# rohanpsingh/LearningHumanoidWalking

Measured on AMD Instinct MI355X. Metric: env-steps/s (whole job): on-device rollout + GAE + PPO update, higher is better.
Workload: dtype f64 physics / f32 networks

## Files before the change

include/lhw.h:

```cpp
#ifndef LHW_H
#define LHW_H

#include <stdint.h>

#include "lhw_model_fields.h"

#ifdef __cplusplus
extern "C" {
#endif

typedef enum {
  LHW_OK = 0,
  LHW_ERR_ARG = -1,
  LHW_ERR_HIP = -2,
  LHW_ERR_MODEL = -3,
  LHW_ERR_UNSUPPORTED = -4,
  LHW_ERR_NO_DEVICE = -5
} LhwStatus;

typedef enum {
  LHW_TASK_CARTPOLE = 0,
  LHW_TASK_JVRC_WALK = 1,
  LHW_TASK_H1_STAND = 2,
  LHW_TASK_JVRC_STEP = 3,
// ... 279 lines not shown
                       int64_t ws_row, float* mu, float* act, float* logp, float* value, void* stream);
int lhw_ppo_set_inference_dtype(LhwPpo* ppo, int fp16);
int lhw_ppo_set_update_dtype(LhwPpo* ppo, int fp16);
int lhw_ppo_debug_set_strip_fused(LhwPpo* ppo, int32_t on);
int lhw_ppo_debug_set_strip_wide(LhwPpo* ppo, int32_t on);
int lhw_ppo_debug_set_strip_fp16(LhwPpo* ppo, int32_t on);
int lhw_ppo_debug_last_grad_fused(const LhwPpo* ppo);
int lhw_ppo_debug_plan(const LhwPpo* ppo, int32_t B, int32_t imitation, int32_t* out13);
int lhw_gae(int32_t T, int32_t N, const float* rew, const float* val, const uint8_t* done, const float* vterm,
            const float* vfinal, double gamma, double lam, float* ret, float* adv, void* stream);
int lhw_moments(const float* x, int64_t n, double* out2_dev, void* stream);
int lhw_scale_shift(float* x, int64_t n, float mean, float inv_scale, void* stream);
int lhw_standardize(float* x, int64_t n, const double* stats3_dev, double eps, void* stream);
int lhw_ppo_set_imitation(LhwPpo* ppo, const float* target, const uint8_t* mask, float coeff, int64_t n_selected);
int lhw_ppo_grad(LhwPpo* ppo, const float* theta, float* grad, const float* xn, const float* xm, const float* act,
                 const float* old_logp, const float* adv, const float* ret, const int32_t* idx, int32_t B,
                 float* stats_dev, void* stream);
int lhw_ppo_apply(LhwPpo* ppo, float* theta, float* grad, float* adam_m, float* adam_v, int64_t step, float grad_scale,
                  void* stream);
int lhw_ppo_debug_grad_sqnorms(LhwPpo* ppo, float* out2_host);
int lhw_ppo_step(LhwPpo* ppo, float* theta, float* grad, float* adam_m, float* adam_v, const float* xn, const float* xm, const float* act,
                 const float* old_logp, const float* adv, const float* ret, const int32_t* idx, int32_t B, float* stats_dev, int64_t step,
                 float grad_scale, void* stream);

typedef struct LhwRnn LhwRnn;
int lhw_rnn_create(const LhwPpoConfig* cfg, int32_t seq_len, int32_t seq_cols, int32_t rollout_rows, LhwRnn** out);
int lhw_rnn_destroy(LhwRnn* rnn);
int64_t lhw_rnn_param_count(const LhwRnn* rnn);
int lhw_rnn_layout(const LhwRnn* rnn, int64_t* out19);
int lhw_rnn_forward(LhwRnn* rnn, const float* theta, const float* obs, int64_t N, const float* obs_mean, const float* obs_std,
                    const uint8_t* reset, uint64_t seed, uint32_t env_id_base, uint32_t counter, int deterministic, int commit,
                    float* mu, float* act, float* logp, float* value, void* stream);
int lhw_rnn_values(LhwRnn* rnn, const float* theta, const float* obs, const float* term_obs, const uint8_t* done,
                   const uint8_t* reset0, int32_t T, int32_t N, const float* obs_mean, const float* obs_std,
                   float* val, float* vterm, float* vfinal, void* stream);
int lhw_rnn_rollout_policy(LhwRnn* rnn, const float* theta, const float* obs_mean, const float* obs_std, uint64_t seed, uint32_t counter,
                           int deterministic, LhwRolloutLstmPolicy* out, void* stream);
int lhw_rnn_grad(LhwRnn* rnn, const float* theta, float* grad, int32_t T, int32_t N, const float* xn, const float* xm,
                 const float* act, const float* old_logp, const float* adv, const float* ret, const uint8_t* done,
                 const int32_t* cols, int32_t B, float* stats_dev, void* stream);
int lhw_rnn_apply(LhwRnn* rnn, float* theta, float* grad, float* adam_m, float* adam_v, int64_t step, float grad_scale,
                  void* stream);
#define LHW_LSTM_SEQ_MIN_HIDDEN 32
#define LHW_LSTM_SEQ_MAX_HIDDEN 256
#define LHW_LSTM_SEQ_MAX_OBS_PAD 128
#define LHW_ROLLOUT_HISTORY_MAX_OBS_PAD 1024
// ... 38 lines not shown
```

learninghumanoidwalking_amd/_lib.py:

```python
from __future__ import annotations

import ctypes
import glob
import os
import subprocess

import numpy as np

_HERE = os.path.dirname(os.path.abspath(__file__))
_ROOT = os.path.dirname(_HERE)
LIB_PATH = os.environ.get("LHW_LIB") or os.path.join(_HERE, "liblhw.so")
_LIB = None


class LhwError(RuntimeError):
    def __init__(self, code, msg):
        super().__init__(f"liblhw error {code}: {msg}")
        self.code = code


class LhwEnvConfig(ctypes.Structure):
    _fields_ = [
        ("task", ctypes.c_int32), ("n_envs", ctypes.c_int32), ("device", ctypes.c_int32),
        ("frame_skip", ctypes.c_int32), ("max_traj_len", ctypes.c_int32), ("env_id_base", ctypes.c_int32),
# ... 324 lines not shown
    sig("lhw_ppo_debug_last_grad_fused", [vp])
    sig("lhw_ppo_debug_plan", [vp, i32, i32, ctypes.POINTER(i32)])
    sig("lhw_debug_wgrad_wide", [vp, vp, i32, i32, vp, vp, vp])
    sig("lhw_debug_wgrad_skinny", [i32, i32, i32, i32, vp, vp, i32, vp, vp, i32, vp, vp, vp, vp, vp, vp])
    sig("lhw_debug_dpp_forms", [u64, vp, vp, vp, vp])
    sig("lhw_debug_fastmath", [i64, vp, vp, vp, vp, vp, vp, vp])
    sig("lhw_env_phase_cycles", [vp, ctypes.c_int, vp])
    sig("lhw_env_step_range", [vp, i32, i32, vp, vp, vp, vp, vp, vp, vp])
    sig("lhw_ppo_create", [ctypes.POINTER(LhwPpoConfig), ctypes.POINTER(vp)])
    sig("lhw_ppo_destroy", [vp])
    sig("lhw_ppo_param_count", [vp], i64)
    sig("lhw_ppo_layout", [vp, ctypes.POINTER(i64)])
    sig("lhw_ppo_normalize", [vp, vp, i64, vp, vp, vp, vp, vp])
    sig("lhw_ppo_forward", [vp, vp, vp, i64, vp, vp, u64, u32, u32, ctypes.c_int, vp, vp, vp, vp, vp])
    sig("lhw_ppo_forward_at", [vp, vp, vp, i64, vp, vp, u64, u32, u32, ctypes.c_int, i64, vp, vp, vp, vp, vp])
    sig("lhw_ppo_begin_rollout", [vp, vp, vp])
    sig("lhw_ppo_end_rollout", [vp])
    sig("lhw_ppo_set_inference_dtype", [vp, ctypes.c_int])
    sig("lhw_ppo_set_update_dtype", [vp, ctypes.c_int])
    sig("lhw_ppo_set_imitation", [vp, vp, vp, f32, i64])
    sig("lhw_ppo_grad", [vp, vp, vp, vp, vp, vp, vp, vp, vp, vp, i32, vp, vp])
    sig("lhw_ppo_apply", [vp, vp, vp, vp, vp, i64, f32, vp])
    sig("lhw_ppo_step", [vp, vp, vp, vp, vp, vp, vp, vp, vp, vp, vp, vp, i32, vp, i64, f32, vp])
    sig("lhw_ppo_debug_grad_sqnorms", [vp, ctypes.POINTER(f32)])
    sig("lhw_gae", [i32, i32, vp, vp, vp, vp, vp, ctypes.c_double, ctypes.c_double, vp, vp, vp])
    sig("lhw_moments", [vp, i64, vp, vp])
    sig("lhw_scale_shift", [vp, i64, f32, f32, vp])
    sig("lhw_standardize", [vp, i64, vp, ctypes.c_double, vp])
    sig("lhw_rnn_create", [ctypes.POINTER(LhwPpoConfig), i32, i32, i32, ctypes.POINTER(vp)])
    sig("lhw_rnn_destroy", [vp])
    sig("lhw_rnn_param_count", [vp], i64)
    sig("lhw_rnn_layout", [vp, ctypes.POINTER(i64)])
    sig("lhw_rnn_normalize", [vp, vp, i64, vp, vp, vp, vp, vp])
    sig("lhw_rnn_forward", [vp, vp, vp, i64, vp, vp, vp, u64, u32, u32, ctypes.c_int, ctypes.c_int, vp, vp, vp, vp, vp])
    sig("lhw_rnn_grad", [vp, vp, vp, i32, i32, vp, vp, vp, vp, vp, vp, vp, vp, i32, vp, vp])
    sig("lhw_rnn_apply", [vp, vp, vp, vp, vp, i64, f32, vp])
    sig("lhw_rnn_debug_grad_sqnorms", [vp, ctypes.POINTER(f32)])
    sig("lhw_rnn_debug_set_seq_fused", [vp, i32])
    sig("lhw_rnn_debug_last_grad_fused", [vp])
    sig("lhw_debug_lstm_seq", [ctypes.POINTER(LhwLstmSeqArgs), i32, vp])
    sig("lhw_debug_lstm_values", [ctypes.POINTER(LhwLstmValuesArgs), i32, vp])
    sig("lhw_rnn_values", [vp, vp, vp, vp, vp, vp, i32, i32, vp, vp, vp, vp, vp, vp])
    sig("lhw_env_debug_step_record", [vp, vp, vp, vp])
    sig("lhw_env_rollout", [vp, ctypes.POINTER(LhwRolloutPolicy), i32, i32, i32, vp, vp, vp, vp, vp, vp, vp, vp])
    sig("lhw_env_last_rollout_queued", [vp])
    sig("lhw_env_rollout_task_inputs", [vp, ctypes.POINTER(LhwRolloutPolicy), i32, i32, i32, vp, vp, vp, vp, vp, vp, vp, vp, vp])
# ... 39 lines not shown
```

learninghumanoidwalking_amd/csrc/lhw_learner.h:

```cpp
#pragma once
#include "lhw_internal.h"

struct LearnerCore {
  int device = 0, D = 0, Dp = 0, A = 0, H = 0, learn_std = 0;
  float clip, ent_coeff, mirror_coeff, grad_clip, lr, adam_eps, beta1, beta2;
  int use_mirror = 0;
  size_t off_actor = 0, off_std = 0, off_critic = 0, n_critic = 0, n_params = 0;
  int *d_obs_src = nullptr, *d_act_src = nullptr;
  float *d_obs_sign = nullptr, *d_act_sign = nullptr;
  float *stats = nullptr;
  float *stats_part = nullptr;
  float *norm_part = nullptr;
  LhwDevMem mem;
};
#define SUMSQ_BLOCKS 128

int learner_check(const LhwPpoConfig* c, void** out, bool caps_ok);
void learner_init(LearnerCore& k, const LhwPpoConfig* c, size_t n_actor, size_t n_critic);
bool learner_mirror(LearnerCore& k, const LhwPpoConfig* c);
int learner_normalize(LearnerCore* k, const float* obs, int64_t R, const float* obs_mean, const float* obs_std, float* xn, float* xm, void* stream);
int learner_apply(LearnerCore* k, float* theta, float* grad, float* adam_m, float* adam_v, int64_t step, float grad_scale, void* stream);
int learner_grad_sqnorms(LearnerCore* k, float* out2_host);

struct AdamArgs {
  float *theta, *grad, *m, *v;
  size_t n0, off1, n1;
  int blocks0;
  float gscale;
  float* part;
  float* normsq_out;
  float max_norm, lr, beta1, beta2, eps, bc1, bc2sqrt;
};
AdamArgs learner_adam_args(const LearnerCore& k, float* theta, float* grad, float* adam_m, float* adam_v, int64_t step, float grad_scale);
__global__ void adam2_kernel(AdamArgs a);

struct StreamPair {
  hipStream_t s, sc;
  hipEvent_t ev_fork, ev_join;
  void fork() const { if (sc != s) { (void)hipEventRecord(ev_fork, s); (void)hipStreamWaitEvent(sc, ev_fork, 0); } }
  void join() const { if (sc != s) { (void)hipEventRecord(ev_join, sc); (void)hipStreamWaitEvent(s, ev_join, 0); } }
};

__global__ void normalize_kernel(const float* __restrict__ obs, int D, int Dp, size_t R, const float* __restrict__ mean, const float* __restrict__ stdv,
                                 float* __restrict__ xn, float* __restrict__ xm, const int* __restrict__ src, const float* __restrict__ sign);
__global__ void sample_kernel(const float* __restrict__ mu, int ldmu, int A, int N, const float* __restrict__ stdv, uint64_t seed, uint32_t env_base,
                              uint32_t counter, int deterministic, float* __restrict__ act, float* __restrict__ logp);
__global__ void ppo_loss_kernel(int B, int Rcap, int A, int Op, const float* __restrict__ ya, const float* __restrict__ yc, const float* __restrict__ act,
                                const float* __restrict__ old_logp, const float* __restrict__ adv, const float* __restrict__ ret,
                                const float* __restrict__ stdv, float clip, float mirror_coeff, int use_mirror, const int* __restrict__ act_src,
                                const float* __restrict__ act_sign, float* __restrict__ dya, float* __restrict__ dyc, float* __restrict__ dstd,
                                float* __restrict__ stats_part, const float* __restrict__ imit_target, const unsigned char* __restrict__ imit_mask,
                                float imit_coeff, float imit_inv_count, int seqB, float gscale);
__global__ void ppo_stats_rows_kernel(int B, int A, const float* __restrict__ rows, int ld, float imit_inv_count, float* __restrict__ stats_part);
__global__ void reduce_rows_kernel(const float* __restrict__ part, int nrows, int n, float* __restrict__ out);
__global__ void entropy_grad_kernel(const float* __restrict__ stdv, int A, float ent_coeff, float* __restrict__ grad_std);
```

learninghumanoidwalking_amd/csrc/lhw_learner.hip:

```cpp
#include "lhw_learner.h"

#include <cmath>
#include <mutex>
#include <vector>

#include "lhw_policy.h"
#include "lhw_rng.h"

__global__ void normalize_kernel(const float* __restrict__ obs, int D, int Dp, size_t R, const float* __restrict__ mean,
                                 const float* __restrict__ stdv, float* __restrict__ xn, float* __restrict__ xm,
                                 const int* __restrict__ src, const float* __restrict__ sign) {
  size_t i = (size_t)blockIdx.x * blockDim.x + threadIdx.x;
  if (i >= R * (size_t)Dp) return;
  size_t r = i / Dp;
  int j = (int)(i - r * Dp);
  float v = 0.f, vm = 0.f;
  if (j < D) {
    v = (obs[r * D + j] - mean[j]) / stdv[j];
    if (xm) vm = (sign[j] * obs[r * D + src[j]] - mean[j]) / stdv[j];
  }
  xn[i] = v;
  if (xm) xm[i] = vm;
}
__global__ void __launch_bounds__(256) sample_kernel(const float* __restrict__ mu, int ldmu, int A, int N, const float* __restrict__ stdv,
// ... 59 lines not shown
                                                             float* __restrict__ stats_part) {
  const int m = blockIdx.x * blockDim.x + threadIdx.x;
  float t[NSTAT] = {0, 0, 0, 0, 0, 0};
  if (m < B)
    for (int k = 0; k < NSTAT; k++) t[k] = rows[(size_t)k * ld + m];
  const float invB = 1.f / (float)B, invBA = 1.f / ((float)B * (float)A);
  float vals[NSTAT] = {t[0] * invB, t[1] * invB, t[2] * invBA, t[3] * invB, t[4] * invB, t[5] * imit_inv_count};
  ppo_stats_block(vals, stats_part);
}

__global__ void reduce_rows_kernel(const float* __restrict__ part, int nrows, int n, float* __restrict__ out) {
  int k = threadIdx.x;
  if (k >= n) return;
  float s = 0.f;
  for (int b = 0; b < nrows; b++) s += part[(size_t)b * n + k];
  out[k] += s;
}

__global__ void entropy_grad_kernel(const float* __restrict__ stdv, int A, float ent_coeff, float* __restrict__ grad_std) {
  int a = threadIdx.x;
  if (a < A) grad_std[a] += -ent_coeff / ((float)A * stdv[a]);
}
__global__ void __launch_bounds__(256) sumsq2_kernel(const float* __restrict__ g0, size_t n0, const float* __restrict__ g1, size_t n1, float scale,
                                                     float* __restrict__ part ) {
  const int grp = blockIdx.x / SUMSQ_BLOCKS, b = blockIdx.x - grp * SUMSQ_BLOCKS;
  const float* __restrict__ g = grp ? g1 : g0;
  const size_t n = grp ? n1 : n0;
  float s = 0.f;
  for (size_t i = (size_t)b * blockDim.x + threadIdx.x; i < n; i += (size_t)SUMSQ_BLOCKS * blockDim.x) {
    float v = g[i] * scale;
    s += v * v;
  }
  for (int o = 32; o > 0; o >>= 1) s += __shfl_xor(s, o);
  __shared__ float red[4];
  LHW_LDS_POISON(red);
  if ((threadIdx.x & 63) == 0) red[threadIdx.x >> 6] = s;
  __syncthreads();
  if (threadIdx.x == 0) part[blockIdx.x] = (red[0] + red[1]) + (red[2] + red[3]);
}
__global__ void __launch_bounds__(256) adam2_kernel(AdamArgs a) {
  float *__restrict__ theta = a.theta, *__restrict__ grad = a.grad, *__restrict__ m = a.m, *__restrict__ v = a.v, *__restrict__ normsq_out = a.normsq_out;
  const float* __restrict__ part = a.part;
  const size_t n0 = a.n0, off1 = a.off1, n1 = a.n1;
  const int blocks0 = a.blocks0;
  const float gscale = a.gscale, max_norm = a.max_norm, lr = a.lr, beta1 = a.beta1, beta2 = a.beta2, eps = a.eps, bc1 = a.bc1, bc2sqrt = a.bc2sqrt;
  const int grp = (int)blockIdx.x >= blocks0 ? 1 : 0;
  __shared__ float nsq;
  LHW_LDS_POISON(nsq);
  if (threadIdx.x == 0) {
    float s = 0.f;
    for (int b = 0; b < SUMSQ_BLOCKS; b++) s += part[grp * SUMSQ_BLOCKS + b];
    nsq = s;
    if ((int)blockIdx.x == (grp ? blocks0 : 0)) normsq_out[grp] = s;
  }
  __syncthreads();
  const size_t i = (size_t)((int)blockIdx.x - (grp ? blocks0 : 0)) * blockDim.x + threadIdx.x;
  if (i >= (grp ? n1 : n0)) return;
  const size_t e = (grp ? off1 : 0) + i;
  float norm = sqrtf(nsq);
  float coef = max_norm / (norm + 1e-6f);
  coef = coef < 1.f ? coef : 1.f;
  float g = grad[e] * gscale * coef;
  float mi = beta1 * m[e] + (1.f - beta1) * g;
  float vi = beta2 * v[e] + (1.f - beta2) * g * g;
  m[e] = mi; v[e] = vi;
  float denom = sqrtf(vi) / bc2sqrt + eps;
  theta[e] -= (lr / bc1) * (mi / denom);
  grad[e] = 0.f;
}
__global__ void __launch_bounds__(256) gae_kernel(int T, int N, const float* __restrict__ rew, const float* __restrict__ val,
                                                  const uint8_t* __restrict__ done, const float* __restrict__ vterm,
                                                  const float* __restrict__ vfinal, double gamma, double lam,
                                                  float* __restrict__ ret, float* __restrict__ adv) {
  int n = blockIdx.x * blockDim.x + threadIdx.x;
  if (n >= N) return;
  double gae = 0.0, nextv = (double)vfinal[n];
  for (int t = T - 1; t >= 0; t--) {
    size_t i = (size_t)t * N + n;
    uint8_t f = done[i];
// ... 124 lines not shown
  return LHW_OK;
}
extern "C" int lhw_scale_shift(float* x, int64_t n, float mean, float inv_scale, void* stream) {
  if (!x || n <= 0) return lhw_fail(LHW_ERR_ARG, "bad argument");
  int dev = 0;
  if (device_of(x, &dev)) return LHW_ERR_HIP;
  hipLaunchKernelGGL(scale_shift_kernel, dim3((n + 255) / 256), dim3(256), 0, (hipStream_t)stream, x, (size_t)n, mean, inv_scale);
  HIPCHK(hipGetLastError());
  return LHW_OK;
}

extern "C" int lhw_standardize(float* x, int64_t n, const double* stats3_dev, double eps, void* stream) {
  if (!x || !stats3_dev || n <= 0) return lhw_fail(LHW_ERR_ARG, "bad argument");
  int dev = 0;
  if (device_of(x, &dev)) return LHW_ERR_HIP;
  hipLaunchKernelGGL(standardize_kernel, dim3((n + 255) / 256), dim3(256), 0, (hipStream_t)stream, x, (size_t)n, stats3_dev, eps);
  HIPCHK(hipGetLastError());
  return LHW_OK;
}
AdamArgs learner_adam_args(const LearnerCore& k, float* theta, float* grad, float* adam_m, float* adam_v, int64_t step, float grad_scale) {
  const size_t na = k.learn_std ? k.off_std + k.A : k.off_std;
  const float bc1 = 1.f - powf(k.beta1, (float)step), bc2 = 1.f - powf(k.beta2, (float)step);
  return AdamArgs{theta, grad, adam_m, adam_v, na, k.off_critic, k.n_critic, (int)((na + 255) / 256), grad_scale, k.norm_part, k.stats + 8,
                  k.grad_clip, k.lr, k.beta1, k.beta2, k.adam_eps, bc1, sqrtf(bc2)};
}
static void clip_and_adam(const AdamArgs& a, hipStream_t s) {
  const int blocks1 = (int)((a.n1 + 255) / 256);
  hipLaunchKernelGGL(sumsq2_kernel, dim3(2 * SUMSQ_BLOCKS), dim3(256), 0, s, a.grad, a.n0, a.grad + a.off1, a.n1, a.gscale, a.part);
  hipLaunchKernelGGL(adam2_kernel, dim3(a.blocks0 + blocks1), dim3(256), 0, s, a);
}

int learner_apply(LearnerCore* k, float* theta, float* grad, float* adam_m, float* adam_v, int64_t step, float grad_scale, void* stream) {
  if (!k || !theta || !grad || !adam_m || !adam_v || step <= 0) return lhw_fail(LHW_ERR_ARG, "bad argument");
  HIPCHK(hipSetDevice(k->device));
  hipStream_t s = (hipStream_t)stream;
  clip_and_adam(learner_adam_args(*k, theta, grad, adam_m, adam_v, step, grad_scale), s);
  if (!k->learn_std) HIPCHK(hipMemsetAsync(grad + k->off_std, 0, sizeof(float) * pad4(k->A), s));
  HIPCHK(hipGetLastError());
  return LHW_OK;
}

int learner_grad_sqnorms(LearnerCore* k, float* out2_host) {
  if (!k || !out2_host) return lhw_fail(LHW_ERR_ARG, "null argument");
  HIPCHK(hipSetDevice(k->device));
  HIPCHK(hipDeviceSynchronize());
  HIPCHK(hipMemcpy(out2_host, k->stats + 8, 2 * sizeof(float), hipMemcpyDeviceToHost));
  return LHW_OK;
}
```

learninghumanoidwalking_amd/csrc/lhw_ppo.hip:

```cpp
#include <hip/hip_runtime.h>

#include <cmath>
#include <cstdlib>
#include <cstring>
#include <memory>
#include <vector>

#include "lhw_gemm.h"
#include "lhw_learner.h"
#include "lhw_mlp_strip_h.h"

struct MlpLayout {
  int D, Dp, H, O, Op;
  size_t w1, b1, w2, b2, w3, b3, total;
};
static MlpLayout mlp_layout(int D, int H, int O) {
  MlpLayout L;
  L.D = D; L.Dp = pad4(D); L.H = H; L.O = O; L.Op = pad4(O);
  size_t o = 0;
  L.w1 = o; o += (size_t)H * L.Dp;
  L.b1 = o; o += H;
  L.w2 = o; o += (size_t)H * H;
  L.b2 = o; o += H;
  L.w3 = o; o += (size_t)L.Op * H;
  L.b3 = o; o += L.Op;
  L.total = o;
  return L;
}
struct StripWeights { const float *w1t, *b1, *w2t, *b2, *w3t, *b3; };
static StripWeights strip_weights(const MlpLayout& L, const float* wt, const float* th) {
  const float* w2t = wt + (size_t)L.Dp * L.H;
  return {wt, th + L.b1, w2t, th + L.b2, w2t + (size_t)L.H * L.H, th + L.b3};
}
static void strip_h_prepare(const MlpLayout& L, const float* th, _Float16* wh, hipStream_t s) { mlp_strip_h_prepare(th + L.w1, th + L.w2, th + L.w3, L.Dp, L.O, wh, s); }
static void strip_prepare(const MlpLayout& L, const float* th, float* wt, hipStream_t s) { mlp_strip_prepare(th + L.w1, th + L.w2, th + L.w3, L.Dp, L.O, L.Op, wt, s); }
struct MlpNet {
  MlpLayout L;
  const float* x = nullptr; int ldx = 0;
  float *h1 = nullptr, *h2 = nullptr, *y = nullptr;
  float *dy = nullptr, *dh2 = nullptr, *dh1 = nullptr;
  float* wt = nullptr;
  unsigned *bits1 = nullptr, *bits2 = nullptr;
  const _Float16* x_h = nullptr; int ldxh = 0;
  _Float16 *h1_h = nullptr, *h2_h = nullptr, *dh2_h = nullptr, *dh1_h = nullptr;
  _Float16* wh = nullptr;
};
struct RowSpan { size_t first; int rows; };
struct Switches {
  int mlp_strip;
  int strip_bits, strip_fused;
  int strip_wide;
  int two_streams, graph, fp16_storage;
  int strip_fp16;
};
static Switches read_switches() {
  auto on = [](const char* name, int dflt) { const char* v = getenv(name); return v ? atoi(v) : dflt; };
  return {on("LHW_MLP_STRIP", 2), on("LHW_STRIP_BITS", 1) != 0, on("LHW_STRIP_FUSED", 1) != 0, 0, on("LHW_PPO_TWO_STREAMS", 1) != 0,
          on("LHW_PPO_GRAPH", 1) != 0, on("LHW_FP16_STORAGE", 1) != 0, 0};
}
struct UpdatePlan {
  int32_t half, hstore;
  int32_t fwd_strip, bwd_strip;
  int32_t train;
  int32_t bits, wide;
  int32_t streams;
};
struct InferPlan {
  int32_t half, strips, policy_step;
  int32_t critic_copies, actor_copies;
};
struct MlpPass {
  int half = 0; bool hstore = false;
  const float* wt = nullptr;
  const _Float16* wh = nullptr;
  bool keep = false, bits = false;
  bool bwd_strip = false, have_dh = false;
};
struct StepKey {
  const void* ptr[12]; int32_t B; uint32_t gs; UpdatePlan plan;
  bool operator==(const StepKey& o) const { return memcmp(this, &o, sizeof o) == 0; }
};
static_assert(std::has_unique_object_representations_v<StepKey>, "StepKey is compared as bytes");

struct LhwPpo : LearnerCore {
  int max_rows;
  _Float16* xb_h = nullptr; int ldxh = 0;
  int infer_half = 0, update_half = 0;
  MlpNet a, c;
  float *xb = nullptr;
  float *mb_act = nullptr, *mb_logp = nullptr, *mb_adv = nullptr, *mb_ret = nullptr;
  float *part = nullptr;
  float *dstd = nullptr;
  float *wt_inf = nullptr;
  float *wt_roll = nullptr;
  _Float16 *wh_inf = nullptr, *wh_roll = nullptr;
  const float* roll_theta = nullptr;
  const float* imit_target = nullptr; const unsigned char* imit_mask = nullptr;
  float imit_coeff = 0.f, imit_inv_count = 0.f;
  float *bwd_part = nullptr;
  int max_slices = 0;
  hipStream_t side = nullptr;
  hipEvent_t ev_fork = nullptr, ev_join = nullptr, ev_head = nullptr;
  Switches sw{};
  float* stat_rows = nullptr;
  UpdatePlan last_plan{};
  hipGraph_t step_graph = nullptr; hipGraphExec_t step_exec = nullptr; hipGraphNode_t node_gather = nullptr, node_adam = nullptr;
  StepKey step_key{};
  ~LhwPpo() {
    (void)hipSetDevice(device);
    if (step_exec) (void)hipGraphExecDestroy(step_exec);
    if (step_graph) (void)hipGraphDestroy(step_graph);
    if (side) { (void)hipStreamSynchronize(side); (void)hipStreamDestroy(side); }
    for (hipEvent_t e : {ev_fork, ev_join, ev_head}) if (e) (void)hipEventDestroy(e);
  }
};
#define WT_SLOTS 8
static bool rollout_wide_supported(const MlpLayout& L) {
  return L.H == 256 && L.Dp > 64 && L.Dp <= LHW_ROLLOUT_HISTORY_MAX_OBS_PAD && (L.Dp & 3) == 0 && L.O > 0 && L.O <= 32 && L.Op >= L.O;
}
static bool strip_shape(const MlpLayout& L, bool wide_on) {
  return mlp_strip_supported(L.H, L.Dp, L.O, L.Op) || (wide_on && mlp_strip_wide_supported(L.H, L.Dp, L.O, L.Op));
}
static bool strip_h_shape(const MlpLayout& L) { return mlp_strip_h_supported(L.H, L.Dp, L.O, L.Op); }
static bool train_strip_shape(const MlpLayout& L, int critic, bool wide_on) {
  return mlp_train_strip_supported(L.H, L.Dp, L.O, L.Op, critic) || (wide_on && mlp_train_strip_wide_supported(L.H, L.Dp, L.O, L.Op, critic));
}
static UpdatePlan update_plan(const LhwPpo* p, bool imitation) {
  const Switches& w = p->sw;
  UpdatePlan u{};
  u.half = p->update_half; u.hstore = u.half && p->xb_h != nullptr;
  auto takes = [&](const MlpLayout& L) { return u.half ? strip_h_shape(L) : strip_shape(L, w.strip_wide); };
  const int nets = w.mlp_strip >= 1 && (!u.half || (u.hstore && w.strip_fp16 && p->a.wh)) ? (takes(p->a.L) ? 1 : 0) | (takes(p->c.L) ? 2 : 0) : 0;
  u.train = nets == 3 && !u.half && w.strip_fused && !imitation && train_strip_shape(p->a.L, 0, w.strip_wide) && train_strip_shape(p->c.L, 1, w.strip_wide);
  u.fwd_strip = u.bwd_strip = u.train ? 0 : nets;
  u.bits = u.fwd_strip && !u.half && p->a.bits1 != nullptr;
  u.wide = nets && !strip_shape(p->c.L, false);
// ... 517 lines not shown
    HIPCHK(hipGraphGetNodes(g, nullptr, &nn));
    std::vector<hipGraphNode_t> nodes(nn);
    HIPCHK(hipGraphGetNodes(g, nodes.data(), &nn));
    for (hipGraphNode_t nd : nodes) {
      hipGraphNodeType ty;
      if (hipGraphNodeGetType(nd, &ty) != hipSuccess || ty != hipGraphNodeTypeKernel) continue;
      hipKernelNodeParams kp;
      if (hipGraphKernelNodeGetParams(nd, &kp) != hipSuccess) continue;
      if (kp.func == (void*)gather_kernel) p->node_gather = nd;
      else if (kp.func == (void*)adam2_kernel) p->node_adam = nd;
    }
    if (!p->node_gather || !p->node_adam) return lhw_fail(LHW_ERR_HIP, "lhw_ppo_step: gather / Adam nodes not found in the captured graph (%zu nodes)", nn);
    HIPCHK(hipGraphInstantiate(&p->step_exec, g, nullptr, nullptr, 0));
    p->step_key = key;
  }
  GatherArgs ga = gather_args(p, xn, xm, act, old_logp, adv, ret, idx, B);
  AdamArgs aa = learner_adam_args(*p, theta, grad, adam_m, adam_v, step, grad_scale);
  if (const int rc = patch_kernel_arg(p->step_exec, p->node_gather, &ga)) return rc;
  if (const int rc = patch_kernel_arg(p->step_exec, p->node_adam, &aa)) return rc;
  p->roll_theta = nullptr;
  HIPCHK(hipGraphLaunch(p->step_exec, s));
  return LHW_OK;
}
```

learninghumanoidwalking_amd/ppo.py:

```python
from __future__ import annotations

import datetime
import os
import sys
import time
from dataclasses import dataclass
from pathlib import Path

import numpy as np
import torch

from . import _lib, dist_utils
from .batched_env import REWARD_TERMS, TASK_JVRC_STEP, term_stats_dict
from .ppo_kernels import PpoKernels, reference_init
from .task_hook import reward_only_on


@dataclass
class BatchData:
    states: torch.Tensor
    actions: torch.Tensor
    rewards: torch.Tensor
    values: torch.Tensor
    returns: torch.Tensor
# ... 660 lines not shown
        adv = self._adv.reshape(-1)
        self._normalize_advantages(adv)
        ret = self._ret.reshape(-1)
        raw_obs = ro.obs[:T].reshape(n_samples, -1)
        xn, xm = k.normalize(raw_obs)
        act = ro.act.reshape(n_samples, -1)
        logp = ro.logp.reshape(-1)
        if getattr(k, "inference_fp16", False) and not getattr(k, "update_fp16", False):
            logp = self._float32_log_probs(raw_obs, act)
        mb = int(self.minibatch_size or n_samples)
        mb = min(mb, n_samples)
        k.stats.zero_()
        n_updates = 0
        fused = (self.imitation_projector is None and not dist_utils._active(dist_utils.dist())
                 and os.environ.get("LHW_PPO_GRAPH", "1") != "0")
        cur = torch.cuda.current_stream(self.device)
        if fused:
            if getattr(self, "_update_stream", None) is None:
                self._update_stream = torch.cuda.Stream(device=self.device)
            self._update_stream.wait_stream(cur)
        with torch.cuda.stream(self._update_stream if fused else cur):
            for epoch in range(self.epochs):
                perm = self._minibatch_perm(itr, epoch, n_samples)
                for start in range(0, n_samples - mb + 1, mb):
                    mb_idx = perm[start:start + mb]
                    if fused:
                        k.step_minibatch(xn, xm, act, logp, adv, ret, mb_idx)
                    else:
                        imit = self._imitation_term(raw_obs.index_select(0, mb_idx.long())) if self.imitation_projector is not None else None
                        k.grad_minibatch(xn, xm, act, logp, adv, ret, mb_idx, imitation=imit)
                        self._allreduce_and_apply()
                    n_updates += 1
        if fused:
            cur.wait_stream(self._update_stream)
        s = (k.stats / max(1, n_updates)).cpu().numpy()
        self.last_losses = dict(actor=float(s[0]), critic=float(s[1]), mirror=float(s[2]), kl=float(s[3]),
                                clip_fraction=float(s[4]), imitation=float(s[5]), entropy=self._entropy_penalty(), n_updates=n_updates)
        return self.last_losses

    def _minibatch_perm(self, itr, epoch, n_samples, rank=None):
        g = torch.Generator(device=self.device)
        base = self.seed if self.seed is not None else 0
        g.manual_seed(base + itr * self.epochs + epoch + 1000003 * (self.rank if rank is None else rank))
        return torch.randperm(n_samples, generator=g, device=self.device, dtype=torch.int64).to(torch.int32)

    def _float32_log_probs(self, obs_flat, act_flat):
        k = self.kernels
# ... 124 lines not shown
```

learninghumanoidwalking_amd/ppo_kernels.py:

```python
from __future__ import annotations

import ctypes
import os

import numpy as np
import torch

from . import _lib

def _p(t):
    return ctypes.c_void_p(t.data_ptr()) if t is not None else None


class _Kernels:

    recurrent = False
    _API = "lhw_ppo"

    def __init__(self, obs_dim, act_dim, hidden, max_rows, create_args=(), *, device=0, learn_std=False, lr=3e-4, eps=1e-5,
                 clip=0.2, entropy_coeff=0.0, mirror_coeff=0.4, max_grad_norm=0.5, mirror_obs=None, mirror_act=None):
        if not torch.cuda.is_available():
            raise _lib.LhwError(-5, "no GPU visible: the PPO kernels have no CPU fallback")
        self.device = torch.device("cuda", device) if isinstance(device, int) else device
        self._L = _lib.lib()
# ... 190 lines not shown
        rc = self._L.lhw_ppo_rollout_policy(self._h, _p(self.theta), _p(self.obs_mean), _p(self.obs_std), int(seed) & (2**64 - 1),
                                            int(counter) & 0xFFFFFFFF, int(bool(deterministic)), ctypes.byref(view))
        if rc == -4:
            return None
        _lib.check(rc)
        return view

    def grad_minibatch(self, xn, xm, act, old_logp, adv, ret, idx, imitation=None):
        B = idx.numel()
        if imitation is not None:
            coeff, target, mask, count = imitation
            assert target.shape == (B, self.act_dim) and mask.shape == (B, self.act_dim) and mask.dtype == torch.uint8
            self._imit_keep = (target.contiguous(), mask.contiguous())
            _lib.check(self._L.lhw_ppo_set_imitation(self._h, _p(self._imit_keep[0]), _p(self._imit_keep[1]), float(coeff), int(count)))
        _lib.check(self._L.lhw_ppo_grad(self._h, _p(self.theta), _p(self.grad), _p(xn), _p(xm), _p(act), _p(old_logp),
                                        _p(adv), _p(ret), _p(idx), B, _p(self.stats), self._stream()))

    def step_minibatch(self, xn, xm, act, old_logp, adv, ret, idx, grad_scale=1.0):
        self.adam_step += 1
        _lib.check(self._L.lhw_ppo_step(self._h, _p(self.theta), _p(self.grad), _p(self.adam_m), _p(self.adam_v), _p(xn), _p(xm), _p(act),
                                        _p(old_logp), _p(adv), _p(ret), _p(idx), idx.numel(), _p(self.stats), self.adam_step,
                                        float(grad_scale), self._stream()))


def reference_init(obs_dim, act_dim, hidden=256, init_std=0.223, generator_seed=None):
    import torch.nn as nn

    with torch.random.fork_rng(devices=[]):
        if generator_seed is not None:
            torch.default_generator.manual_seed(int(generator_seed))
        return _reference_init_draw(obs_dim, act_dim, hidden, init_std)


def _reference_init_draw(obs_dim, act_dim, hidden, init_std):
    import torch.nn as nn

    def net(out_dim, scale_out):
        layers = [nn.Linear(obs_dim, hidden), nn.Linear(hidden, hidden), nn.Linear(hidden, out_dim)]
        for l in layers:
            l.weight.data.normal_(0, 1)
            l.weight.data *= 1 / torch.sqrt(l.weight.data.pow(2).sum(1, keepdim=True))
            l.bias.data.fill_(0)
        if scale_out is not None:
            layers[2].weight.data.mul_(scale_out)
        return layers

# ... 10 lines not shown
```

Baseline: 4.278 million.

## Schedule PPO minibatch steps as overlapping actor/critic chains across three streams

Adds lhw_ppo_update_steps, which issues all minibatch updates of an epoch in one call. Actor and critic each run on their own stream, and a third stream gathers minibatches ahead into a ring of buffers. Events order the dependencies, and clip+Adam is split per parameter group so each net updates independently. The aim is to remove per-minibatch host launch/graph overhead and the serialization between actor and critic, at the cost of extra ring buffers and a more complex event schedule.

```diff
diff --git a/include/lhw.h b/include/lhw.h
--- a/include/lhw.h
+++ b/include/lhw.h
@@ -325,6 +325,12 @@
 int lhw_ppo_step(LhwPpo* ppo, float* theta, float* grad, float* adam_m, float* adam_v, const float* xn, const float* xm, const float* act,
                  const float* old_logp, const float* adv, const float* ret, const int32_t* idx, int32_t B, float* stats_dev, int64_t step,
                  float grad_scale, void* stream);
+int lhw_ppo_update_steps(LhwPpo* ppo, float* theta, float* grad, float* adam_m, float* adam_v, const float* xn, const float* xm, const float* act,
+                         const float* old_logp, const float* adv, const float* ret, const int32_t* perm, int32_t B, int32_t n_steps,
+                         float* stats_dev, int64_t step, float grad_scale, void* stream);
+int lhw_ppo_debug_set_chains(LhwPpo* ppo, int32_t on, int32_t lead);
+int lhw_ppo_debug_get_chains(const LhwPpo* ppo, int32_t* out2);
+int lhw_ppo_debug_chain_schedule(int32_t n_steps, int32_t lead, int32_t learn_std, int32_t* out, int32_t max_ops);
 
 typedef struct LhwRnn LhwRnn;
 int lhw_rnn_create(const LhwPpoConfig* cfg, int32_t seq_len, int32_t seq_cols, int32_t rollout_rows, LhwRnn** out);
diff --git a/learninghumanoidwalking_amd/_lib.py b/learninghumanoidwalking_amd/_lib.py
--- a/learninghumanoidwalking_amd/_lib.py
+++ b/learninghumanoidwalking_amd/_lib.py
@@ -370,6 +370,10 @@
     sig("lhw_ppo_grad", [vp, vp, vp, vp, vp, vp, vp, vp, vp, vp, i32, vp, vp])
     sig("lhw_ppo_apply", [vp, vp, vp, vp, vp, i64, f32, vp])
     sig("lhw_ppo_step", [vp, vp, vp, vp, vp, vp, vp, vp, vp, vp, vp, vp, i32, vp, i64, f32, vp])
+    sig("lhw_ppo_update_steps", [vp, vp, vp, vp, vp, vp, vp, vp, vp, vp, vp, vp, i32, i32, vp, i64, f32, vp])
+    sig("lhw_ppo_debug_set_chains", [vp, i32, i32])
+    sig("lhw_ppo_debug_get_chains", [vp, ctypes.POINTER(i32)])
+    sig("lhw_ppo_debug_chain_schedule", [i32, i32, i32, ctypes.POINTER(i32), i32])
     sig("lhw_ppo_debug_grad_sqnorms", [vp, ctypes.POINTER(f32)])
     sig("lhw_gae", [i32, i32, vp, vp, vp, vp, vp, ctypes.c_double, ctypes.c_double, vp, vp, vp])
     sig("lhw_moments", [vp, i64, vp, vp])
diff --git a/learninghumanoidwalking_amd/csrc/lhw_learner.h b/learninghumanoidwalking_amd/csrc/lhw_learner.h
--- a/learninghumanoidwalking_amd/csrc/lhw_learner.h
+++ b/learninghumanoidwalking_amd/csrc/lhw_learner.h
@@ -30,9 +30,11 @@
   float* part;
   float* normsq_out;
   float max_norm, lr, beta1, beta2, eps, bc1, bc2sqrt;
+  int block_first;
 };
 AdamArgs learner_adam_args(const LearnerCore& k, float* theta, float* grad, float* adam_m, float* adam_v, int64_t step, float grad_scale);
 __global__ void adam2_kernel(AdamArgs a);
+void clip_and_adam_group(const AdamArgs& a, int grp, hipStream_t s);
 
 struct StreamPair {
   hipStream_t s, sc;
diff --git a/learninghumanoidwalking_amd/csrc/lhw_learner.hip b/learninghumanoidwalking_amd/csrc/lhw_learner.hip
--- a/learninghumanoidwalking_amd/csrc/lhw_learner.hip
+++ b/learninghumanoidwalking_amd/csrc/lhw_learner.hip
@@ -105,8 +105,9 @@
   if (a < A) grad_std[a] += -ent_coeff / ((float)A * stdv[a]);
 }
 __global__ void __launch_bounds__(256) sumsq2_kernel(const float* __restrict__ g0, size_t n0, const float* __restrict__ g1, size_t n1, float scale,
-                                                     float* __restrict__ part ) {
-  const int grp = blockIdx.x / SUMSQ_BLOCKS, b = blockIdx.x - grp * SUMSQ_BLOCKS;
+                                                     float* __restrict__ part , int block_first) {
+  const int bid = (int)blockIdx.x + block_first;
+  const int grp = bid / SUMSQ_BLOCKS, b = bid - grp * SUMSQ_BLOCKS;
   const float* __restrict__ g = grp ? g1 : g0;
   const size_t n = grp ? n1 : n0;
   float s = 0.f;
@@ -119,7 +120,7 @@
   LHW_LDS_POISON(red);
   if ((threadIdx.x & 63) == 0) red[threadIdx.x >> 6] = s;
   __syncthreads();
-  if (threadIdx.x == 0) part[blockIdx.x] = (red[0] + red[1]) + (red[2] + red[3]);
+  if (threadIdx.x == 0) part[bid] = (red[0] + red[1]) + (red[2] + red[3]);
 }
 __global__ void __launch_bounds__(256) adam2_kernel(AdamArgs a) {
   float *__restrict__ theta = a.theta, *__restrict__ grad = a.grad, *__restrict__ m = a.m, *__restrict__ v = a.v, *__restrict__ normsq_out = a.normsq_out;
@@ -127,17 +128,18 @@
   const size_t n0 = a.n0, off1 = a.off1, n1 = a.n1;
   const int blocks0 = a.blocks0;
   const float gscale = a.gscale, max_norm = a.max_norm, lr = a.lr, beta1 = a.beta1, beta2 = a.beta2, eps = a.eps, bc1 = a.bc1, bc2sqrt = a.bc2sqrt;
-  const int grp = (int)blockIdx.x >= blocks0 ? 1 : 0;
+  const int bid = (int)blockIdx.x + a.block_first;
+  const int grp = bid >= blocks0 ? 1 : 0;
   __shared__ float nsq;
   LHW_LDS_POISON(nsq);
   if (threadIdx.x == 0) {
     float s = 0.f;
     for (int b = 0; b < SUMSQ_BLOCKS; b++) s += part[grp * SUMSQ_BLOCKS + b];
     nsq = s;
-    if ((int)blockIdx.x == (grp ? blocks0 : 0)) normsq_out[grp] = s;
-  }
-  __syncthreads();
-  const size_t i = (size_t)((int)blockIdx.x - (grp ? blocks0 : 0)) * blockDim.x + threadIdx.x;
+    if (bid == (grp ? blocks0 : 0)) normsq_out[grp] = s;
+  }
+  __syncthreads();
+  const size_t i = (size_t)(bid - (grp ? blocks0 : 0)) * blockDim.x + threadIdx.x;
   if (i >= (grp ? n1 : n0)) return;
   const size_t e = (grp ? off1 : 0) + i;
   float norm = sqrtf(nsq);
@@ -308,12 +310,19 @@
   const size_t na = k.learn_std ? k.off_std + k.A : k.off_std;
   const float bc1 = 1.f - powf(k.beta1, (float)step), bc2 = 1.f - powf(k.beta2, (float)step);
   return AdamArgs{theta, grad, adam_m, adam_v, na, k.off_critic, k.n_critic, (int)((na + 255) / 256), grad_scale, k.norm_part, k.stats + 8,
-                  k.grad_clip, k.lr, k.beta1, k.beta2, k.adam_eps, bc1, sqrtf(bc2)};
+                  k.grad_clip, k.lr, k.beta1, k.beta2, k.adam_eps, bc1, sqrtf(bc2), 0};
 }
 static void clip_and_adam(const AdamArgs& a, hipStream_t s) {
   const int blocks1 = (int)((a.n1 + 255) / 256);
-  hipLaunchKernelGGL(sumsq2_kernel, dim3(2 * SUMSQ_BLOCKS), dim3(256), 0, s, a.grad, a.n0, a.grad + a.off1, a.n1, a.gscale, a.part);
+  hipLaunchKernelGGL(sumsq2_kernel, dim3(2 * SUMSQ_BLOCKS), dim3(256), 0, s, a.grad, a.n0, a.grad + a.off1, a.n1, a.gscale, a.part, 0);
   hipLaunchKernelGGL(adam2_kernel, dim3(a.blocks0 + blocks1), dim3(256), 0, s, a);
+}
+void clip_and_adam_group(const AdamArgs& a, int grp, hipStream_t s) {
+  AdamArgs g = a;
+  g.block_first = grp ? a.blocks0 : 0;
+  const int blocks = grp ? (int)((a.n1 + 255) / 256) : a.blocks0;
+  hipLaunchKernelGGL(sumsq2_kernel, dim3(SUMSQ_BLOCKS), dim3(256), 0, s, a.grad, a.n0, a.grad + a.off1, a.n1, a.gscale, a.part, grp ? SUMSQ_BLOCKS : 0);
+  hipLaunchKernelGGL(adam2_kernel, dim3(blocks), dim3(256), 0, s, g);
 }
 
 int learner_apply(LearnerCore* k, float* theta, float* grad, float* adam_m, float* adam_v, int64_t step, float grad_scale, void* stream) {
diff --git a/learninghumanoidwalking_amd/csrc/lhw_ppo.hip b/learninghumanoidwalking_amd/csrc/lhw_ppo.hip
--- a/learninghumanoidwalking_amd/csrc/lhw_ppo.hip
+++ b/learninghumanoidwalking_amd/csrc/lhw_ppo.hip
@@ -9,6 +9,7 @@
 #include "lhw_gemm.h"
 #include "lhw_learner.h"
 #include "lhw_mlp_strip_h.h"
+#include "lhw_ppo_chains.h"
 
 struct MlpLayout {
   int D, Dp, H, O, Op;
@@ -52,11 +53,16 @@
   int strip_wide;
   int two_streams, graph, fp16_storage;
   int strip_fp16;
+  int chains, chain_lead;
 };
+#define CHAINS_DEFAULT 1
+#define CHAIN_LEAD_DEFAULT 0
+static int clamp_lead(int lead) { return lead < 0 ? 0 : (lead > CH_MAX_LEAD ? CH_MAX_LEAD : lead); }
 static Switches read_switches() {
   auto on = [](const char* name, int dflt) { const char* v = getenv(name); return v ? atoi(v) : dflt; };
   return {on("LHW_MLP_STRIP", 2), on("LHW_STRIP_BITS", 1) != 0, on("LHW_STRIP_FUSED", 1) != 0, 0, on("LHW_PPO_TWO_STREAMS", 1) != 0,
-          on("LHW_PPO_GRAPH", 1) != 0, on("LHW_FP16_STORAGE", 1) != 0, 0};
+          on("LHW_PPO_GRAPH", 1) != 0, on("LHW_FP16_STORAGE", 1) != 0, 0, on("LHW_PPO_CHAINS", CHAINS_DEFAULT) != 0,
+          clamp_lead(on("LHW_PPO_CHAIN_LEAD", CHAIN_LEAD_DEFAULT))};
 }
 struct UpdatePlan {
   int32_t half, hstore;
@@ -81,6 +87,7 @@
   bool operator==(const StepKey& o) const { return memcmp(this, &o, sizeof o) == 0; }
 };
 static_assert(std::has_unique_object_representations_v<StepKey>, "StepKey is compared as bytes");
+struct ChainSlot { float *xb, *act, *logp, *adv, *ret, *stat_rows; };
 
 struct LhwPpo : LearnerCore {
   int max_rows;
@@ -106,12 +113,17 @@
   UpdatePlan last_plan{};
   hipGraph_t step_graph = nullptr; hipGraphExec_t step_exec = nullptr; hipGraphNode_t node_gather = nullptr, node_adam = nullptr;
   StepKey step_key{};
+  hipStream_t aux = nullptr;
+  hipEvent_t ev_chain[CH_EV_KINDS * CH_RING] = {};
+  ChainSlot chain_slots[CH_MAX_LEAD + 2] = {};
   ~LhwPpo() {
     (void)hipSetDevice(device);
     if (step_exec) (void)hipGraphExecDestroy(step_exec);
     if (step_graph) (void)hipGraphDestroy(step_graph);
     if (side) { (void)hipStreamSynchronize(side); (void)hipStreamDestroy(side); }
+    if (aux) { (void)hipStreamSynchronize(aux); (void)hipStreamDestroy(aux); }
     for (hipEvent_t e : {ev_fork, ev_join, ev_head}) if (e) (void)hipEventDestroy(e);
+    for (hipEvent_t e : ev_chain) if (e) (void)hipEventDestroy(e);
   }
 };
 #define WT_SLOTS 8
@@ -675,3 +687,125 @@
   HIPCHK(hipGraphLaunch(p->step_exec, s));
   return LHW_OK;
 }
+static int chains_setup(LhwPpo* p, int depth) {
+  if (!p->aux) HIPCHK(hipStreamCreateWithFlags(&p->aux, hipStreamNonBlocking));
+  for (hipEvent_t& e : p->ev_chain)
+    if (!e) HIPCHK(hipEventCreateWithFlags(&e, hipEventDisableTiming));
+  p->chain_slots[0] = ChainSlot{p->xb, p->mb_act, p->mb_logp, p->mb_adv, p->mb_ret, p->stat_rows};
+  const size_t R = p->max_rows;
+  for (int i = 1; i < depth; i++) {
+    if (p->chain_slots[i].xb) continue;
+    const size_t mark = p->mem.mark();
+    ChainSlot c{p->mem.get<float>(2 * R * p->a.L.Dp), p->mem.get<float>(R * p->A), p->mem.get<float>(R), p->mem.get<float>(R), p->mem.get<float>(R),
+                p->mem.get<float>((size_t)NSTAT * R)};
+    if (p->mem.failed()) {
+      p->mem.release_to(mark);
+      return lhw_fail(LHW_ERR_HIP, "lhw_ppo_update_steps: ring slot %d of the minibatch buffers: allocation failed (max_rows=%d)", i, p->max_rows);
+    }
+    p->chain_slots[i] = c;
+  }
+  return LHW_OK;
+}
+extern "C" int lhw_ppo_update_steps(LhwPpo* p, float* theta, float* grad, float* adam_m, float* adam_v, const float* xn, const float* xm, const float* act,
+                                    const float* old_logp, const float* adv, const float* ret, const int32_t* perm, int32_t B, int32_t n_steps,
+                                    float* stats_dev, int64_t step, float grad_scale, void* stream) {
+  if (!p || !theta || !grad || !adam_m || !adam_v || !xn || !act || !old_logp || !adv || !ret || !perm || !stats_dev || step <= 0 || n_steps <= 0)
+    return lhw_fail(LHW_ERR_ARG, "bad argument");
+  if (B <= 0 || B > p->max_rows) return lhw_fail(LHW_ERR_ARG, "minibatch %d exceeds workspace capacity %d", B, p->max_rows);
+  const UpdatePlan u = update_plan(p, p->imit_target != nullptr);
+  if (!p->sw.chains || !u.train || u.streams != 2 || p->imit_target != nullptr)
+    return lhw_fail(LHW_ERR_UNSUPPORTED, "lhw_ppo_update_steps: %s", !p->sw.chains ? "switched off (LHW_PPO_CHAINS)" : p->imit_target ? "an imitation term is armed"
+                    : !u.train ? "the update's plan has no train strips" : "one stream (LHW_PPO_TWO_STREAMS=0)");
+  HIPCHK(hipSetDevice(p->device));
+  const int lead = p->sw.chain_lead;
+  if (const int rc = chains_setup(p, chain_depth(lead))) return rc;
+  p->last_plan = u;
+  p->roll_theta = nullptr;
+  const int mir = p->use_mirror && xm != nullptr;
+  const MlpLayout &La = p->a.L, &Lc = p->c.L;
+  const int R = p->max_rows, Dp = La.Dp, Op = La.Op;
+  const float *th_a = theta + p->off_actor, *th_c = theta + p->off_critic;
+  const RowSpans spans = actor_spans(mir, B, R); const RowSpan rows_c{0, B};
+  const BwdParts Pa = bwd_parts_carve(La, R, 2, p->bwd_part);
+  const BwdParts Pc = bwd_parts_carve(Lc, R, 1, p->bwd_part + bwd_parts_floats(La, R, 2));
+  MlpPass pass; pass.keep = true; pass.have_dh = true;
+  const int nblk = (B + 255) / 256;
+  BwdSlices z[2];
+  const hipStream_t streams[CH_STREAMS] = {(hipStream_t)stream, p->side, p->aux};
+  for (const ChainOp& o : chain_schedule(n_steps, lead, p->learn_std != 0)) {
+    const hipStream_t q = streams[o.stream];
+    const ChainSlot& sl = p->chain_slots[o.slot >= 0 ? o.slot : 0];
+    const bool critic = o.net == CH_CRITIC;
+    switch (o.kind) {
+      case CH_WAIT: HIPCHK(hipStreamWaitEvent(q, p->ev_chain[o.event], 0)); break;
+      case CH_RECORD: HIPCHK(hipEventRecord(p->ev_chain[o.event], q)); break;
+      case CH_GATHER: {
+        GatherArgs g = gather_args(p, xn, xm, act, old_logp, adv, ret, perm + (size_t)o.step * B, B);
+        g.xb = sl.xb; g.mact = sl.act; g.mlogp = sl.logp; g.madv = sl.adv; g.mret = sl.ret;
+        hipLaunchKernelGGL(gather_kernel, dim3(((size_t)B * Dp + 255) / 256), dim3(256), 0, q, g);
+        break;
+      }
+      case CH_PREPARE:
+        if (critic) strip_prepare(Lc, th_c, p->c.wt, q); else strip_prepare(La, th_a, p->a.wt, q);
+        break;
+      case CH_STRIP: {
+        const MlpNet& n = critic ? p->c : p->a;
+        const MlpLayout& L = n.L;
+        const float* th = critic ? th_c : th_a;
+        const LhwPpoHead head{B, p->A, Op, sl.act, sl.logp, sl.adv, sl.ret, theta + p->off_std, p->clip, p->mirror_coeff, mir, p->d_act_src,
+                              p->d_act_sign, p->learn_std ? p->dstd : (float*)nullptr, nullptr, nullptr, 0.f, 0.f, 1.f};
+        const StripWeights w = strip_weights(L, n.wt, th);
+        MlpStripTrain t{MlpStripFwd{w.w1t, w.b1, w.w2t, w.b2, w.w3t, w.b3, sl.xb, Dp, L.Dp, L.O, L.Op, B, n.h1, n.h2, nullptr},
+                        th + L.w2, th + L.w3, n.dy, n.dh2, n.dh1, critic ? 0 : (mir ? R : 0), critic ? 1 : 0, head, sl.stat_rows, R};
+        mlp_train_strip(t, q);
+        break;
+      }
+      case CH_STD_GRAD:
+        colsum_det(p->dstd, B, Op, p->A, grad + p->off_std, p->part, q);
+        hipLaunchKernelGGL(entropy_grad_kernel, dim3(1), dim3(64), 0, q, theta + p->off_std, p->A, p->ent_coeff, grad + p->off_std);
+        break;
+      case CH_WGRAD: {
+        MlpNet n = critic ? p->c : p->a;
+        n.x = sl.xb;
+        z[o.net] = BwdSlices{};
+        if (critic) mlp_backward(n, th_c, rows_c, Pc, z[o.net], q, pass);
+        else for (int i = 0; i < spans.n; i++) mlp_backward(n, th_a, spans.v[i], Pa, z[o.net], q, pass);
+        break;
+      }
+      case CH_REDUCE: {
+        SegList S; S.n = 0; S.scale = 1.f;
+        if (critic) mlp_backward_segments(S, Lc, grad + p->off_critic, Pc, z[o.net]); else mlp_backward_segments(S, La, grad + p->off_actor, Pa, z[o.net]);
+        launch_reduce_segments(S, q);
+        break;
+      }
+      case CH_CLIP_ADAM: clip_and_adam_group(learner_adam_args(*p, theta, grad, adam_m, adam_v, step + o.step, grad_scale), o.net, q); break;
+      case CH_ZERO_STD: HIPCHK(hipMemsetAsync(grad + p->off_std, 0, sizeof(float) * pad4(p->A), q)); break;
+      case CH_STATS:
+        hipLaunchKernelGGL(ppo_stats_rows_kernel, dim3(nblk), dim3(256), 0, q, B, p->A, sl.stat_rows, R, p->imit_inv_count, p->stats_part);
+        hipLaunchKernelGGL(reduce_rows_kernel, dim3(1), dim3(64), 0, q, p->stats_part, nblk, NSTAT, stats_dev);
+        break;
+      default: return lhw_fail(LHW_ERR_ARG, "lhw_ppo_update_steps: unknown op %d in the schedule", o.kind);
+    }
+  }
+  HIPCHK(hipGetLastError());
+  return LHW_OK;
+}
+extern "C" int lhw_ppo_debug_set_chains(LhwPpo* p, int32_t on, int32_t lead) {
+  if (!p || lead > CH_MAX_LEAD) return lhw_fail(LHW_ERR_ARG, "bad argument (lead %d, at most %d)", lead, CH_MAX_LEAD);
+  p->sw.chains = on ? 1 : 0;
+  if (lead >= 0) p->sw.chain_lead = lead;
+  return LHW_OK;
+}
+extern "C" int lhw_ppo_debug_get_chains(const LhwPpo* p, int32_t* out2) {
+  if (!p || !out2) return lhw_fail(LHW_ERR_ARG, "null argument");
+  out2[0] = p->sw.chains; out2[1] = p->sw.chain_lead;
+  return LHW_OK;
+}
+extern "C" int lhw_ppo_debug_chain_schedule(int32_t n_steps, int32_t lead, int32_t learn_std, int32_t* out, int32_t max_ops) {
+  if (n_steps <= 0 || lead < 0 || lead > CH_MAX_LEAD || max_ops < 0 || (max_ops > 0 && !out)) return lhw_fail(LHW_ERR_ARG, "bad argument");
+  const std::vector<ChainOp> ops = chain_schedule(n_steps, lead, learn_std != 0);
+  static_assert(sizeof(ChainOp) == CH_OP_WORDS * sizeof(int32_t), "ChainOp is handed out as CH_OP_WORDS int32");
+  const size_t n = std::min<size_t>(ops.size(), (size_t)max_ops);
+  if (n) memcpy(out, ops.data(), n * sizeof(ChainOp));
+  return (int)ops.size();
+}
diff --git a/learninghumanoidwalking_amd/csrc/lhw_ppo_chains.h b/learninghumanoidwalking_amd/csrc/lhw_ppo_chains.h
--- /dev/null
+++ b/learninghumanoidwalking_amd/csrc/lhw_ppo_chains.h
@@ -0,0 +1,80 @@
+#pragma once
+#include <stdint.h>
+
+#include <vector>
+
+#define CH_MAX_LEAD 4
+#define CH_RING 8
+enum { CH_MAIN = 0, CH_SIDE = 1, CH_AUX = 2, CH_STREAMS = 3 };
+enum { CH_ACTOR = 0, CH_CRITIC = 1 };
+enum {
+  CH_WAIT = 0, CH_RECORD = 1,
+  CH_GATHER = 2,
+  CH_PREPARE = 3,
+  CH_STRIP = 4,
+  CH_STD_GRAD = 5,
+  CH_WGRAD = 6,
+  CH_REDUCE = 7,
+  CH_CLIP_ADAM = 8,
+  CH_ZERO_STD = 9,
+  CH_STATS = 10
+};
+enum {
+  CH_EV_START = 0, CH_EV_GATHER = 1, CH_EV_A_STRIP = 2, CH_EV_C_STRIP = 3, CH_EV_A_BWD = 4, CH_EV_C_BWD = 5, CH_EV_A_DONE = 6, CH_EV_C_DONE = 7,
+  CH_EV_END_SIDE = 8, CH_EV_END_AUX = 9, CH_EV_KINDS = 10
+};
+struct ChainOp { int32_t kind, stream, step, net, slot, event; };
+#define CH_OP_WORDS 6
+
+static inline int chain_depth(int lead) { return lead + 2; }
+static inline int chain_event(int kind, int step) { return kind * CH_RING + (step % CH_RING + CH_RING) % CH_RING; }
+
+static inline std::vector<ChainOp> chain_schedule(int n_steps, int lead, bool learn_std) {
+  std::vector<ChainOp> ops;
+  if (n_steps <= 0 || lead < 0 || lead > CH_MAX_LEAD) return ops;
+  const int G = chain_depth(lead);
+  auto op = [&](int kind, int stream, int step, int net, int event) { ops.push_back(ChainOp{kind, stream, step, net, step >= 0 ? step % G : -1, event}); };
+  auto wait = [&](int stream, int evkind, int step) { op(CH_WAIT, stream, step, -1, chain_event(evkind, step)); };
+  auto record = [&](int stream, int evkind, int step) { op(CH_RECORD, stream, step, -1, chain_event(evkind, step)); };
+  auto gather = [&](int j) {
+    if (j >= n_steps) return;
+    if (j >= G) { wait(CH_AUX, CH_EV_A_BWD, j - G); wait(CH_AUX, CH_EV_C_BWD, j - G); }
+    op(CH_GATHER, CH_AUX, j, -1, -1);
+    record(CH_AUX, CH_EV_GATHER, j);
+  };
+  auto chain = [&](int k, int net) {
+    const int st = net == CH_ACTOR ? CH_MAIN : CH_SIDE;
+    if (lead == 0) { if (k > 0) wait(st, net == CH_ACTOR ? CH_EV_C_DONE : CH_EV_A_DONE, k - 1); }
+    else if (net == CH_CRITIC && k - lead >= 0) wait(st, CH_EV_A_BWD, k - lead);
+    wait(st, CH_EV_GATHER, k);
+    op(CH_STRIP, st, k, net, -1);
+    record(st, net == CH_ACTOR ? CH_EV_A_STRIP : CH_EV_C_STRIP, k);
+    if (net == CH_ACTOR && learn_std) op(CH_STD_GRAD, st, k, net, -1);
+    op(CH_WGRAD, st, k, net, -1);
+    record(st, net == CH_ACTOR ? CH_EV_A_BWD : CH_EV_C_BWD, k);
+    op(CH_REDUCE, st, k, net, -1);
+    op(CH_CLIP_ADAM, st, k, net, -1);
+    if (net == CH_ACTOR && !learn_std) op(CH_ZERO_STD, st, k, net, -1);
+    op(CH_PREPARE, st, k, net, -1);
+    if (lead == 0) record(st, net == CH_ACTOR ? CH_EV_A_DONE : CH_EV_C_DONE, k);
+  };
+  record(CH_MAIN, CH_EV_START, 0);
+  wait(CH_SIDE, CH_EV_START, 0);
+  wait(CH_AUX, CH_EV_START, 0);
+  op(CH_PREPARE, CH_SIDE, -1, CH_CRITIC, -1);
+  op(CH_PREPARE, CH_MAIN, -1, CH_ACTOR, -1);
+  for (int j = 0; j <= lead; j++) gather(j);
+  for (int k = 0; k < n_steps; k++) {
+    gather(k + lead + 1);
+    chain(k, CH_CRITIC);
+    chain(k, CH_ACTOR);
+    wait(CH_AUX, CH_EV_A_STRIP, k);
+    wait(CH_AUX, CH_EV_C_STRIP, k);
+    op(CH_STATS, CH_AUX, k, -1, -1);
+  }
+  record(CH_SIDE, CH_EV_END_SIDE, 0);
+  record(CH_AUX, CH_EV_END_AUX, 0);
+  wait(CH_MAIN, CH_EV_END_SIDE, 0);
+  wait(CH_MAIN, CH_EV_END_AUX, 0);
+  return ops;
+}
diff --git a/learninghumanoidwalking_amd/ppo.py b/learninghumanoidwalking_amd/ppo.py
--- a/learninghumanoidwalking_amd/ppo.py
+++ b/learninghumanoidwalking_amd/ppo.py
@@ -706,7 +706,9 @@
         with torch.cuda.stream(self._update_stream if fused else cur):
             for epoch in range(self.epochs):
                 perm = self._minibatch_perm(itr, epoch, n_samples)
-                for start in range(0, n_samples - mb + 1, mb):
+                done = k.update_steps(xn, xm, act, logp, adv, ret, perm, mb) if fused else 0
+                n_updates += done
+                for start in range(done * mb, n_samples - mb + 1, mb):
                     mb_idx = perm[start:start + mb]
                     if fused:
                         k.step_minibatch(xn, xm, act, logp, adv, ret, mb_idx)
diff --git a/learninghumanoidwalking_amd/ppo_kernels.py b/learninghumanoidwalking_amd/ppo_kernels.py
--- a/learninghumanoidwalking_amd/ppo_kernels.py
+++ b/learninghumanoidwalking_amd/ppo_kernels.py
@@ -236,6 +236,29 @@
                                         _p(old_logp), _p(adv), _p(ret), _p(idx), idx.numel(), _p(self.stats), self.adam_step,
                                         float(grad_scale), self._stream()))
 
+    def set_chains(self, on=True, lead=None):
+        _lib.check(self._L.lhw_ppo_debug_set_chains(self._h, int(bool(on)), -1 if lead is None else int(lead)))
+
+    @property
+    def chains(self):
+        out = (ctypes.c_int32 * 2)()
+        _lib.check(self._L.lhw_ppo_debug_get_chains(self._h, out))
+        return bool(out[0]), int(out[1])
+
+    def update_steps(self, xn, xm, act, old_logp, adv, ret, perm, mb, grad_scale=1.0):
+        n = perm.numel() // int(mb)
+        if n <= 0 or not hasattr(self._L, "lhw_ppo_update_steps"):
+            return 0
+        assert perm.dtype == torch.int32 and perm.is_contiguous()
+        rc = self._L.lhw_ppo_update_steps(self._h, _p(self.theta), _p(self.grad), _p(self.adam_m), _p(self.adam_v), _p(xn), _p(xm), _p(act),
+                                          _p(old_logp), _p(adv), _p(ret), _p(perm), int(mb), n, _p(self.stats), self.adam_step + 1,
+                                          float(grad_scale), self._stream())
+        if rc == -4:
+            return 0
+        _lib.check(rc)
+        self.adam_step += n
+        return n
+
 
 def reference_init(obs_dim, act_dim, hidden=256, init_std=0.223, generator_seed=None):
     import torch.nn as nn
```

New measurement: 4.308 million, median of 6. About the same (+0.7%).
